# Purpurax/mcaat

Hardware: AMD Instinct MI355X
Metric: k-mers/sec through sdbg_build+cycle_finder, 1B-node graph @ 1/2/4/8 GPUs (higher is better)
Workload: dtype u64

## Files before the change

include/mcaat_gpu.h:

```cpp
#ifndef MCAAT_GPU_H
#define MCAAT_GPU_H
#include <stddef.h>
#include <stdint.h>

#ifdef __cplusplus
extern "C" {
#endif

enum mcaat_status {
    MCAAT_OK = 0,
    MCAAT_E_INVALID = -1,
    MCAAT_E_HIP = -2,
    MCAAT_E_NOMEM = -3,
    MCAAT_E_IO = -4,
    MCAAT_E_CAPACITY = -5
};

typedef struct mcaat_ctx mcaat_ctx;
typedef struct mcaat_reads mcaat_reads;
typedef struct mcaat_graph mcaat_graph;
typedef struct mcaat_cycles mcaat_cycles;
typedef struct mcaat_counts mcaat_counts;
typedef struct mcaat_mapped mcaat_mapped;
typedef struct mcaat_comm mcaat_comm;
// ... 90 lines not shown
                     const uint64_t **offsets, size_t *n_cycles);
int mcaat_cycles_export(const mcaat_cycles *c, uint64_t *sizes, uint64_t *starts, uint64_t *entry_offsets,
                        uint64_t *cycle_offsets, uint64_t *nodes);
int mcaat_cycles_stats(const mcaat_cycles *c, uint64_t *stats);
int mcaat_cycles_candidates(const mcaat_cycles *c, size_t *n, const uint64_t **ids, const int32_t **buckets);
void mcaat_cycles_free(mcaat_cycles *c);

#define MCAAT_COMM_ID_BYTES 128
int mcaat_comm_unique_id(uint8_t *id);
int mcaat_comm_init_rccl(mcaat_ctx *ctx, int world, int rank, const uint8_t *id, mcaat_comm **out);
int mcaat_comm_init_shm(mcaat_ctx *ctx, int world, int rank, const char *name, uint64_t slot_bytes,
                        mcaat_comm **out);
int mcaat_comm_info(const mcaat_comm *c, int *world, int *rank);
int mcaat_comm_schedule_check(int world, uint64_t seed, uint64_t piece_bytes, uint64_t *rounds);
int mcaat_desc_canonical(const uint64_t in[2], int E, uint64_t out[2]);
int mcaat_comm_barrier(mcaat_comm *c);
int mcaat_comm_allgather_sizes(mcaat_comm *c, uint64_t bytes, uint64_t *sizes);
int mcaat_comm_allgatherv(mcaat_comm *c, const void *send, uint64_t bytes, void *recv, const uint64_t *sizes);
void mcaat_comm_free(mcaat_comm *c);
int mcaat_reads_from_fastx_part(mcaat_ctx *ctx, const char *const *files, int n_files, int part, int n_parts,
                                mcaat_reads **out);
int mcaat_reads_file_records(const mcaat_reads *r, int file, uint64_t *n_records);
int mcaat_build_graph_sharded(mcaat_ctx *ctx, mcaat_comm *comm, const mcaat_reads *r, int k, mcaat_graph **out);
int mcaat_cycle_finder_comm(mcaat_graph *g, mcaat_comm *comm, const mcaat_cf_params *p, mcaat_cycles **out);
int mcaat_graph_shard_info(const mcaat_graph *g, int *sharded, uint64_t *first, uint64_t *n_local);
int mcaat_graph_unshard(mcaat_graph *g, mcaat_comm *comm);

int mcaat_stage_times(const mcaat_ctx *ctx, int max, const char **names, double *ms, int *n);
int mcaat_kernel_timing(const mcaat_ctx *ctx, const char *kernel, double *avg_ms, uint64_t *launches,
                        double *bytes_per_launch);
// ... 15 lines not shown
```

mcaat_amd/__init__.py:

```python
from .lib import (
    LIB_PATH,
    CfParams,
    Comm,
    Context,
    Counts,
    CycleResult,
    Graph,
    McaatError,
    Reads,
    SynthSpec,
    count_edges,
    desc_canonical,
    desc_preaggregate,
    edges_reduce,
    device_count,
    load_library,
    preload,
    synth_arrays,
    synth_genome_host,
    synth_host,
)
```

mcaat_amd/csrc/capi.hip:

```cpp
#include <sys/stat.h>
#include <zlib.h>

#include <cstdio>
#include <cstdlib>
#include <cstring>
#include <string>

#include "internal.h"
#include "comm.h"
#include "desc_canon.h"
#include "synth.h"

using namespace mcaat;

namespace {

thread_local std::string g_last_error;

template <class F>
int guarded(F &&f) {
    try {
        f();
        return MCAAT_OK;
    } catch (const Error &e) {
// ... 1026 lines not shown

void mcaat_reset_timing(mcaat_ctx *ctx) {
    if (ctx) ctx->kstats.clear();
}

int mcaat_set_knob(mcaat_ctx *ctx, const char *name, int64_t value) {
    static const char *const known[] = {
        "nc.group_budget", "nc.fallback_budget", "nc.out_cap", "nc.l1_slots", "nc.fine_bits",
        "nc.edge_cap",     "nc.desc_cap",        "sort.msd",   "sort.wave_limit", "sort.mid_limit",
        "sort.block_limit", "cf.dls_stack",      "cf.dls_visited", "cf.fc_lock", "cf.fc_relax",
        "cf.fc_out",       "cf.fc_window",       "cf.walk_budget", "sdbg.adj_lds",   "sdbg.adj_cap",       "cf.ruler_mask",
        "nc.overlap",      "sort.l3_counting",   "cf.peel_list_div", "cf.peel_list_cap", "cf.cand_cap",
        "fq.hostpack",     "sort.mid_counting", "nc.big_table", "cf.fused_init", "sort.mid_occ", "cf.scan_u", "cf.prep_batch", "cf.dls_lanes", "dist.oriented",
        "sort.small_mid", "sort.small_limit", "cf.recount", "cf.dls_host",
        "dist.desc",      "cf.compact",         "cf.fresh",   "cf.dls_persist", "nc.split_first", "nc.split_max", "cf.pull_flags", "cf.dls_budget", "nc.grow_early",
        "nc.free_sync", "dist.shard_cf", "dist.ruler_mask", "dist.adj_chunk", "dist.dir_edges", "nc.ahead", "dist.adj_ranges", "dist.win_ranges", "cf.dls_lds", "cf.dls_lds_cap", "dist.segs_at_one", "nc.a_mini", "dist.bfs_sync", "cf.compact_pct", "dist.bfs_block", "dist.bfs_frontier", "dist.res_fixed", "dist.res_batch", "dist.res_block_mb", "dist.walk_block", "dist.walk_batch", "dist.grid_blocks", "dist.preagg"};
    return guarded([&] {
        require(ctx && name, "null argument");
        bool ok = false;
        for (const char *k : known) ok = ok || strcmp(k, name) == 0;
        if (!ok) throw Error(MCAAT_E_INVALID, std::string("unknown knob: ") + name);
        if (value < 0) ctx->knobs.erase(name);
        else ctx->knobs[name] = value;
    });
}

int mcaat_comm_unique_id(uint8_t *id) {
    return guarded([&] {
        require(id != nullptr, "null argument");
        comm_unique_id(id);
    });
// ... 3 lines not shown
    return guarded([&] {
        const uint64_t r = comm_schedule_check(world, seed, piece_bytes);
        if (rounds) *rounds = r;
    });
}

int mcaat_desc_canonical(const uint64_t in[2], int E, uint64_t out[2]) {
    return guarded([&] {
        require(in && out, "null argument");
        require(E >= 1 && E <= kMaxK + 1, "E must be in [1, 31]");
        require((int)((in[1] >> kNShift) & 63) + E - 1 <= kDescBases, "descriptor longer than its base field");
        uint64_t w0 = in[0], w1 = in[1];
        desc_canonical(w0, w1, E);
        out[0] = w0;
        out[1] = w1;
    });
}

int mcaat_comm_init_rccl(mcaat_ctx *ctx, int world, int rank, const uint8_t *id, mcaat_comm **out) {
    return guarded([&] {
        require(ctx && id && out, "null argument");
        require(world >= 1 && rank >= 0 && rank < world, "rank must be in [0, world)");
        mcaat::bind(ctx);
        auto *c = new mcaat_comm;
        try {
            c->c = comm_rccl(ctx, world, rank, id);
        } catch (...) {
            delete c;
            throw;
        }
// ... 183 lines not shown
```

mcaat_amd/csrc/desc_canon.h:

```cpp
#pragma once
#include <stdint.h>

#if defined(__HIPCC__)
#include <hip/hip_runtime.h>
#define MCAAT_DESC_HD __host__ __device__ __forceinline__
#else
#define MCAAT_DESC_HD inline
#endif

namespace mcaat {

constexpr int kDescBases = 54;
constexpr int kNShift = 44;
constexpr int kHShift = 50;
constexpr int kHBits = 14;

static_assert(kDescBases < 64, "a canonical descriptor's w0 is never all ones only while L < 64");

#if defined(__has_builtin)
#if __has_builtin(__builtin_bitreverse32)
#define MCAAT_DESC_BITREV 1
#endif
#endif
MCAAT_DESC_HD uint32_t desc_rev2_32(uint32_t x) {
#ifdef MCAAT_DESC_BITREV
    const uint32_t y = __builtin_bitreverse32(x);
    return ((y >> 1) & 0x55555555u) | ((y << 1) & 0xAAAAAAAAu);
#else
    x = ((x >> 2) & 0x33333333u) | ((x & 0x33333333u) << 2);
    x = ((x >> 4) & 0x0F0F0F0Fu) | ((x & 0x0F0F0F0Fu) << 4);
    x = ((x >> 8) & 0x00FF00FFu) | ((x & 0x00FF00FFu) << 8);
    return (x >> 16) | (x << 16);
// ... 30 lines not shown
```

mcaat_amd/csrc/node_counter.hip:

```cpp
#include <hipcub/hipcub.hpp>

#include <algorithm>
#include <cstdio>
#include <cstdlib>
#include <ctime>
#include <functional>
#include <memory>
#include <mutex>
#include <type_traits>

#include "desc_canon.h"
#include "internal.h"

namespace mcaat {

namespace {

constexpr int kBlock = 256;


struct SkParams {
    int E;
    int m;
    int w;
    int nmax;
    int l2_bits;
    uint64_t salt;
    uint32_t mini;
};

__device__ __forceinline__ uint64_t desc_window(uint64_t w0, uint64_t w1, int i, int E) {
    uint64_t v;
    if (i == 0) v = w0;
    else if (i < 32) v = (w0 >> (2 * i)) | (w1 << (64 - 2 * i));
    else v = w1 >> (2 * (i - 32));
    return v & mask_bits(2 * E);
}

__device__ __forceinline__ uint32_t rev2_32(uint32_t x) {
    x = ((x >> 2) & 0x33333333u) | ((x & 0x33333333u) << 2);
    x = ((x >> 4) & 0x0F0F0F0Fu) | ((x & 0x0F0F0F0Fu) << 4);
    return __builtin_bswap32(x);
}
// ... 163 lines not shown
#pragma unroll
        for (int t = 0; t < kCk; ++t) hm[t] = min(S[t], Pm[t + W - 1 - kCk]);
    } else {
#pragma unroll
        for (int t = 0; t < kCk; ++t) {
            uint32_t v = at(t);
#pragma unroll
            for (int q = 1; q < W; ++q) v = min(v, at(t + q));
            hm[t] = v;
        }
    }
}

constexpr uint32_t kMiniOne = 1024, kMiniShard = 256;
constexpr uint16_t kDeadSub = 0xffff;


#ifndef MCAAT_WB
#define MCAAT_WB 4
#endif
#ifndef MCAAT_APF
#define MCAAT_APF 1
#endif
[[maybe_unused]] constexpr int kAPF = MCAAT_APF;
constexpr int kWB = MCAAT_WB;
#ifndef MCAAT_WPIPE
#define MCAAT_WPIPE 0
#endif
#ifndef MCAAT_CLOSEMASK
#define MCAAT_CLOSEMASK 1
#endif
constexpr bool kWPipe = MCAAT_WPIPE != 0;

constexpr int kPeP = 7, kPePar = 14, kPeLane = 15;

template <int W, bool FULL>
__global__ void __launch_bounds__(kAThreads) k_sk_scatter(const uint64_t *__restrict__ packed, ItemSrc src,
                                                          SkParams P, uint4 *__restrict__ l1_data,
                                                          const uint64_t *__restrict__ l1_base,
                                                          const uint64_t *__restrict__ l1_cap,
                                                          unsigned long long *l1_cursor, uint16_t *__restrict__ l1_sub,
                                                          unsigned long long *prof, unsigned long long *rstate, int rmode) {
    __shared__ uint64_t stage[kStage];
#if !MCAAT_A1HASH
    __shared__ uint8_t stage_l1[kStage];
#endif
    __shared__ uint16_t perm[kStage];
    __shared__ uint64_t sbase[kAWaves][2][64];
    __shared__ uint32_t hist[256];
    __shared__ uint32_t boff[256];
    __shared__ uint32_t bcur[256];
    __shared__ unsigned long long rpos[256];
    __shared__ unsigned long long rlim[256];
    __shared__ uint32_t rleft[256];
    __shared__ uint32_t wtot[kAWaves];
    __shared__ int more_flag[2];

    const int wave = threadIdx.x >> 6, lane = threadIdx.x & 63;
    const int tb = threadIdx.x;
    unsigned long long my_next = 0, my_base = 0;
    uint32_t prev_need = 0;
    unsigned long long *rs = rstate ? rstate + ((uint64_t)blockIdx.x * 256 + (tb & 255)) * 3 : nullptr;
    if (tb < 256) {
        hist[tb] = 0;
        bcur[tb] = 0;
        my_base = l1_base[tb];
        rlim[tb] = my_base + l1_cap[tb];
        if (rmode >= 2) {
            rpos[tb] = rs[0];
            rleft[tb] = (uint32_t)rs[1];
            my_next = rs[2];
        } else {
            rleft[tb] = 0;
            my_next = atomicAdd(&l1_cursor[tb], (unsigned long long)P.mini);
        }
    }
    if (threadIdx.x == 0) more_flag[0] = more_flag[1] = 0;
    __syncthreads();
    uint64_t *seg = stage + __builtin_amdgcn_readfirstlane(wave * kSeg);
#if !MCAAT_A1HASH
    uint8_t *seg_l1 = stage_l1 + wave * kSeg;
#endif
    uint32_t nflush = 0;

    const int sub_shift = kHShift + kHBits - P.l2_bits;
    auto put = [&](int b, uint64_t pos, const uint4 &d) {
        if (pos < rlim[b]) {
            l1_data[pos] = d;
            const uint64_t hi = (uint64_t)d.w << 32;
            l1_sub[pos] = ((d.w >> (kNShift - 32)) & 63) ? (uint16_t)(sub_shift < 64 ? hi >> sub_shift : 0) : kDeadSub;
        }
    };

    const uint64_t n_items = src.fixed_len ? src.n_reads * src.ipr : src.n_items;
    const uint64_t n_batches = (n_items + 63) / 64;
    const uint64_t bstride = (uint64_t)gridDim.x * kAWaves;
    uint64_t batch = (uint64_t)blockIdx.x * kAWaves + wave;
    constexpr bool kFull = FULL;
    const uint32_t mmask = (uint32_t)mask_bits(2 * P.m);
    const uint32_t salt32 = (uint32_t)P.salt;
    const int nmax = P.nmax;

    uint32_t H[3 * kCk];
#if MCAAT_AREG
    uint32_t iw[kItemRegs - 1];
    u64x2 nraw[3] = {{0, 0}, {0, 0}, {0, 0}};
    uint64_t s1 = 0, s2 = 0;
    int np1 = 0, np2 = 0;
#pragma unroll
    for (int i = 0; i < kItemRegs - 1; ++i) iw[i] = 0;
#else
    uint64_t cw[3], pa = 0, pb = 0;
// ... 247 lines not shown
#endif
        tick(1);
        if (lane == 0) wtot[wave] = fill;
        if (lane == 0 && (active || batch < n_batches)) more_flag[nflush & 1] = 1;
        lds_barrier();
        const int more = more_flag[nflush & 1];
        if (threadIdx.x == 0) more_flag[(nflush + 1) & 1] = 0;
        ++nflush;
        tick(2);
        if (tb < 256) {
            rpos[tb] += prev_need;
            rleft[tb] -= prev_need;
            const uint32_t need = hist[tb];
            if (need > rleft[tb]) {
                for (uint32_t z = 0; z < rleft[tb]; ++z) put(tb, rpos[tb] + z, make_uint4(0, 0, 0, 0));
                if (need <= P.mini) {
                    rpos[tb] = my_base + my_next;
                    rleft[tb] = P.mini;
                    my_next = atomicAdd(&l1_cursor[tb], (unsigned long long)P.mini);
                } else {
                    const uint32_t grab = ((need + P.mini - 1) / P.mini) * P.mini;
                    rpos[tb] = my_base + atomicAdd(&l1_cursor[tb], (unsigned long long)grab);
                    rleft[tb] = grab;
                }
            }
            prev_need = need;
        }
        if (wave == 0) {
            const uint4 hv = *(const uint4 *)&hist[4 * lane];
            const uint32_t sum4 = hv.x + hv.y + hv.z + hv.w;
            uint32_t incl = sum4;
#pragma unroll
            for (int o = 1; o < 64; o <<= 1) {
                const uint32_t v = __shfl_up(incl, o);
                if (lane >= o) incl += v;
            }
// ... 3 lines not shown
        lds_barrier();
        if (tb < 256) hist[tb] = 0;
        tick(3);
        for (uint32_t e = lane; e < fill; e += 64) {
#if MCAAT_A1HASH
            const int b = (int)(*(const uint32_t *)(seg + e) >> 24);
#else
            const int b = seg_l1[e];
#endif
            perm[boff[b] + atomicAdd(&bcur[b], 1u)] = (uint16_t)(wave * kSeg + e);
        }
        lds_barrier();
        uint32_t total = 0;
#pragma unroll
        for (int w = 0; w < kAWaves; ++w) total += wtot[w];
        uint64_t q[2][kWB], B0[2][kWB], x[2][kWB][3];
        auto load_batch = [&](auto Sc, uint32_t j0) {
            constexpr int S = decltype(Sc)::value;
#pragma unroll
            for (int k = 0; k < kWB; ++k) {
                const uint32_t j = j0 + k * kAThreads;
                q[S][k] = 0;
                B0[S][k] = 0;
                if (j < total) {
                    const uint32_t i = perm[j];
                    q[S][k] = stage[i];
                    const uint32_t hi = (uint32_t)(q[S][k] >> 32);
                    const uint32_t ln = (hi >> kPeLane) & 63, pr = (hi >> kPePar) & 1;
                    B0[S][k] = sbase[i / kSeg][pr][ln] + ((hi >> kPeP) & 127);
                }
// ... 54 lines not shown
        if (tb < 256) bcur[tb] = 0;
        fill = 0;
        bsf = active ? 1u : 0u;
        lds_barrier();
        tick(4);
        if (!more) break;
    }
    if (tb < 256) {
        rpos[tb] += prev_need;
        rleft[tb] -= prev_need;
    }
    if (rmode == 1 || rmode == 2) {
        if (tb < 256) {
            rs[0] = rpos[tb];
            rs[1] = rleft[tb];
            rs[2] = my_next;
        }
        return;
    }
    __syncthreads();
    for (int pass = 0; pass < 2; ++pass) {
        for (int b = 0; b < 256; ++b)
            for (uint32_t z = threadIdx.x; z < rleft[b]; z += kAThreads) put(b, rpos[b] + z, make_uint4(0, 0, 0, 0));
        __syncthreads();
        if (tb < 256) {
            rpos[tb] = my_base + my_next;
            rleft[tb] = P.mini;
        }
        __syncthreads();
    }
    if (prof && lane == 0)
        for (int i = 0; i < 5; ++i) atomicAdd(&prof[i], tp[i]);
}

typedef void (*SkKernel)(const uint64_t *, ItemSrc, SkParams, uint4 *, const uint64_t *, const uint64_t *,
                         unsigned long long *, uint16_t *, unsigned long long *, unsigned long long *, int);
SkKernel sk_kernel(int w, bool full) {
    if (full) {
        switch (w) {
#define MCAAT_SK(W) \
    case W:         \
        return k_sk_scatter<W, true>;
            MCAAT_SK(9) MCAAT_SK(10) MCAAT_SK(11) MCAAT_SK(12) MCAAT_SK(13) MCAAT_SK(14) MCAAT_SK(15) MCAAT_SK(16)
#undef MCAAT_SK
        }
    } else {
        switch (w) {
#define MCAAT_SK(W) \
    case W:         \
        return k_sk_scatter<W, false>;
            MCAAT_SK(1) MCAAT_SK(2) MCAAT_SK(3) MCAAT_SK(4) MCAAT_SK(5) MCAAT_SK(6) MCAAT_SK(7) MCAAT_SK(8)
            MCAAT_SK(9) MCAAT_SK(10) MCAAT_SK(11) MCAAT_SK(12) MCAAT_SK(13) MCAAT_SK(14) MCAAT_SK(15) MCAAT_SK(16)
#undef MCAAT_SK
        }
    }
    throw Error(MCAAT_E_INVALID, "node_counter: minimizer window out of range");
}

constexpr int kBThreads = 1024;
constexpr uint32_t kChunk = 65536;


#ifndef MCAAT_BLG
#define MCAAT_BLG 4
#endif
constexpr int kLG = MCAAT_BLG;
static_assert(kLG == 2 || kLG == 4, "32-B or 64-B lines");
__device__ __forceinline__ uint32_t round4(uint32_t x) { return (x + kLG - 1) & ~(uint32_t)(kLG - 1); }

__device__ __forceinline__ void chunk_hist(const uint16_t *__restrict__ sub, uint64_t s0, uint32_t n, uint32_t *lh) {
    const uint4 *v = (const uint4 *)(sub + s0);
    const uint32_t n8 = n / 8;
    for (uint32_t i0 = threadIdx.x; i0 < n8; i0 += 4 * kBThreads) {
        uint4 q[4];
#pragma unroll
// ... 44 lines not shown
    }
}

constexpr int kMaxSub = 2048;
#ifndef MCAAT_BPF
#define MCAAT_BPF 2
#endif
constexpr int kBPF = MCAAT_BPF;
#ifndef MCAAT_BCOOP
#define MCAAT_BCOOP 1
#endif
constexpr bool kCoopFlush = MCAAT_BCOOP != 0;

template <bool WEIGHTED>
__global__ void __launch_bounds__(kBThreads) k_l2_scatter(const uint4 *__restrict__ data,
                                                          const uint16_t *__restrict__ sub,
                                                          const uint64_t *chunk_start, const uint32_t *chunk_len,
                                                          const uint32_t *runs, int l2_bits, int E,
                                                          uint4 *__restrict__ out, uint64_t gbase,
                                                          const uint32_t *__restrict__ wgt,
                                                          uint32_t *__restrict__ out_w) {
    __shared__ uint4 buf[kMaxSub * kLG];
    __shared__ uint32_t lb[kMaxSub];
    __shared__ uint32_t lc[kMaxSub];
    __shared__ uint32_t bl[kMaxSub];
    const uint32_t S = 1u << l2_bits;
    const uint64_t c = blockIdx.x;
    for (uint32_t i = threadIdx.x; i < S; i += kBThreads) {
        lb[i] = runs[c * S + i];
        lc[i] = 0;
        bl[i] = 0;
    }
    __syncthreads();
    const uint64_t s0 = chunk_start[c];
    const uint32_t n = chunk_len[c];
    uint32_t v[kBPF];
    uint4 d[kBPF];
#pragma unroll
    for (int j = 0; j < kBPF; ++j) {
        const uint32_t i = j * kBThreads + threadIdx.x;
        v[j] = i < n ? sub[s0 + i] : kDeadSub;
        d[j] = i < n ? data[s0 + i] : make_uint4(0, 0, 0, 0);
    }
    for (uint32_t i00 = 0; i00 < n; i00 += kBPF * kBThreads)
#pragma unroll
    for (int j = 0; j < kBPF; ++j) {
        const uint32_t i0 = i00 + j * kBThreads;
        if (i0 >= n) break;
        const uint32_t cv = v[j];
        uint4 cd = d[j];
        const uint32_t ni = i0 + kBPF * kBThreads + threadIdx.x;
        v[j] = ni < n ? sub[s0 + ni] : kDeadSub;
        if (ni < n) d[j] = data[s0 + ni];
        const bool live = cv != kDeadSub;
        uint32_t r = 0, line = 0;
        bool buffered = false;
        if (live) {
            r = atomicAdd(&lc[cv], 1u);
            line = bl[cv];
            if constexpr (WEIGHTED) out_w[(uint64_t)lb[cv] * kLG + r - gbase] = wgt[s0 + i0 + threadIdx.x];
            uint64_t w0 = (uint64_t)cd.x | ((uint64_t)cd.y << 32), w1 = (uint64_t)cd.z | ((uint64_t)cd.w << 32);
            desc_canonical(w0, w1, E);
            cd = make_uint4((uint32_t)w0, (uint32_t)(w0 >> 32), (uint32_t)w1, (uint32_t)(w1 >> 32));
            buffered = r / kLG == line;
            if (buffered) buf[cv * kLG + (r & (kLG - 1))] = cd;
            else out[(uint64_t)lb[cv] * kLG + r - gbase] = cd;
        }
        lds_barrier();
        uint32_t nline = 0;
// ... 672 lines not shown
                }
            }
            if (lane == 0) wsum[wave] = wtotal;
            __syncthreads();
            if (threadIdx.x == 0) {
                uint32_t t = 0;
                for (int w = 0; w < kPWaves; ++w) {
                    const uint32_t v = wsum[w];
                    wsum[w] = t;
                    t += v;
                }
                obase = t ? atomicAdd(&rcur[b], (unsigned long long)t) : 0;
                if (raw && t) atomicAdd(&stat[0], (unsigned long long)t);
            }
            __syncthreads();
            const int sub_shift = 64 - l2_bits;
            auto put = [&](uint64_t o, const uint4 &dsc, uint32_t wt) {
                if (o < ocap) {
                    out[ob + o] = dsc;
                    out_w[ob + o] = wt;
                    const uint64_t hi = (uint64_t)dsc.w << 32;
                    out_sub[ob + o] = (uint16_t)(sub_shift < 64 ? hi >> sub_shift : 0);
                    wacc += wt;
                }
            };
            uint64_t o = obase + wsum[wave];
            if (!raw) {
#pragma unroll
                for (int j = 0; j < kPSlots; ++j) {
                    if (c[j]) {
                        const int i = threadIdx.x + j * kPThreads;
                        const unsigned long long w0 = dk0[i], w1 = dk1[i];
                        put(o + __popcll(m[j] & below),
                            make_uint4((uint32_t)w0, (uint32_t)(w0 >> 32), (uint32_t)w1, (uint32_t)(w1 >> 32)), c[j]);
                    }
                    o += __popcll(m[j]);
                }
// ... 92 lines not shown
    const int E = k + 1;
    SkParams P;
    P.E = E;
    P.m = std::max(3, std::min(16, E - 8));
    if (E >= 22) P.m = std::max(14, std::min(16, E - 14));
    if (const char *e = getenv("MCAAT_MINI_W")) {
        const int wt = atoi(e);
        if (wt >= 1 && wt <= 16) P.m = std::max(3, std::min(16, E - wt + 1));
    }
    if (P.m > E) P.m = E;
    P.w = E - P.m + 1;
    if (P.w > 16) throw Error(MCAAT_E_INVALID, "node_counter: minimizer window above 16");
    P.nmax = kDescBases - E + 1;
    P.salt = 0x6d696e696d697aULL;
    P.mini = kMiniOne;

    return P;
}

void node_counter(mcaat_ctx *ctx, const mcaat_reads *r, int k, CountResult &out) {
    NcBuckets b;
    if (r->ahead && r->ahead_k == k) {
        b = std::move(*r->ahead);
        r->ahead.reset();
        verbose_mark(ctx, "node_counter.A_ahead");
    } else {
        node_counter_a(ctx, r, k, nullptr, b);
    }
    node_counter_bc(ctx, b, k, out);
}

// ... 39 lines not shown
            hipLaunchKernelGGL(k_sum_u32, dim3(grid_for(n_items, kBlock, (unsigned)ctx->n_cu * 8)), dim3(kBlock), 0, st,
                               item_np.p, n_items, socc.p);
            LAUNCH_OK();
            unsigned long long h = 0;
            HIP_OK(hipMemcpyAsync(&h, socc.p, 8, hipMemcpyDeviceToHost, st));
            HIP_OK(hipStreamSynchronize(st));
            n_occ = h;
        }
        src.item_base = item_base.p;
        src.item_np = item_np.p;
        src.n_items = n_items;
    }
    const int fine_bits = pick ? pick(n_occ) : nc_fine_bits(ctx, n_occ);
    P.l2_bits = fine_bits - 8;
    if (pick) P.mini = kMiniShard;
    if (knob_set(ctx, "nc.a_mini")) P.mini = (uint32_t)std::max<int64_t>(8, knob(ctx, "nc.a_mini", 1024)) & ~7u;
    bk.l2_bits = P.l2_bits;
    bk.n_occ = n_occ;
    bk.regions.assign(256, {});
    if (n_occ == 0) {
        bk.data.alloc(1);
        bk.sub.alloc(8);
        return;
    }

    const double dens = 2.0 / (P.w + 1);
    uint64_t est = (uint64_t)(1.08 * (dens * (double)n_occ + (double)n_items)) + 4096;
    std::vector<uint64_t> cap(256), base(257);
    const uint64_t a_grid = (uint64_t)kAPerCu * ctx->n_cu;
    for (int b = 0; b < 256; ++b) cap[b] = (est / 256 + 2 * a_grid * P.mini + 7) & ~7ull;
    if (const int64_t fixed = knob(ctx, "nc.l1_slots", 0))
        for (int b = 0; b < 256; ++b) cap[b] = ((uint64_t)fixed + 7) & ~7ull;
    DevBuf<uint64_t> dcap(256), dbase(257);
    DevBuf<unsigned long long> dcur(256);
    DevBuf<uint4> &l1 = bk.data;
    DevBuf<uint16_t> &l1s = bk.sub;
    std::vector<unsigned long long> tot(256);
    static const bool prof_a = getenv("MCAAT_PROF_A") && getenv("MCAAT_PROF_A")[0] == '1';
    DevBuf<unsigned long long> dprof(8);
    if (prof_a) HIP_OK(hipMemsetAsync(dprof.p, 0, dprof.bytes(), st));
    for (int attempt = 0;; ++attempt) {
        base[0] = 0;
        for (int b = 0; b < 256; ++b) base[b + 1] = base[b] + cap[b];
        l1.alloc(base[256]);
        l1s.alloc(base[256]);
        HIP_OK(hipMemcpyAsync(dcap.p, cap.data(), 8 * 256, hipMemcpyHostToDevice, st));
        HIP_OK(hipMemcpyAsync(dbase.p, base.data(), 8 * 257, hipMemcpyHostToDevice, st));
        HIP_OK(hipMemsetAsync(dcur.p, 0, dcur.bytes(), st));
        {
            KernelTimer kt(ctx, "sk_scatter", 0.0);
            hipLaunchKernelGGL(sk_kernel(P.w, P.m == 16), dim3((unsigned)a_grid), dim3(kAThreads), 0, st, r->packed.p, src, P, l1.p,
                               dbase.p, dcap.p, dcur.p, l1s.p, prof_a ? dprof.p : nullptr, nullptr, 0);
            LAUNCH_OK();
            kt.stop();
        }
        HIP_OK(hipMemcpyAsync(tot.data(), dcur.p, 8 * 256, hipMemcpyDeviceToHost, st));
        HIP_OK(hipStreamSynchronize(st));
        bool ok = true;
        for (int b = 0; b < 256; ++b)
            if (tot[b] > cap[b]) ok = false;
        if (ok) break;
        if (attempt > 0) throw Error(MCAAT_E_CAPACITY, "node_counter: L1 bucket sizing failed");
        for (int b = 0; b < 256; ++b) cap[b] = (tot[b] + 8) & ~7ull;
    }
    uint64_t n_desc = 0;
    bk.base = base;
    for (int b = 0; b < 256; ++b) {
        n_desc += tot[b];
        if (tot[b]) bk.regions[b].push_back({base[b], tot[b]});
    }
    ctx->kstats["sk_scatter"].total_bytes += 0.25 * (double)r->n_bases + 18.0 * (double)n_desc;
    if (prof_a) {
        unsigned long long hp[8];
        HIP_OK(hipMemcpy(hp, dprof.p, 64, hipMemcpyDeviceToHost));
        const double waves = (double)a_grid * kAWaves;
        fprintf(stderr, "[mcaat] pass A per-wave ms (100 MHz clock): scan %.1f bucket %.1f wait %.1f reserve %.1f write %.1f\n",
                hp[0] / waves / 1e5, hp[1] / waves / 1e5, hp[2] / waves / 1e5, hp[3] / waves / 1e5, hp[4] / waves / 1e5);
    }
    verbose_mark(ctx, "node_counter.A");
}

struct NcAhead {
    mcaat_ctx *ctx = nullptr;
    int k = 0;
    SkParams P{};
    uint64_t a_grid = 0;
// ... 6 lines not shown
    bool failed = false, ended = false;
    uint64_t n_occ = 0;
    ~NcAhead() {
        if (ctx && !ended) (void)hipStreamSynchronize(ctx->side);
    }
};

static_assert(kItem == kNcItem, "the packer's item estimate uses pass A's item length");

std::shared_ptr<NcAhead> nc_ahead_begin(mcaat_ctx *ctx, int k, uint64_t n_occ_est, uint64_t n_items_est) {
    auto a = std::make_shared<NcAhead>();
    a->ctx = ctx;
    a->k = k;
    a->P = sk_params(k);
    a->P.l2_bits = nc_fine_bits(ctx, n_occ_est) - 8;
    if (knob_set(ctx, "nc.a_mini")) a->P.mini = (uint32_t)std::max<int64_t>(8, knob(ctx, "nc.a_mini", 1024)) & ~7u;
    a->bk = std::make_shared<NcBuckets>();
    a->bk->l2_bits = a->P.l2_bits;
    a->a_grid = (uint64_t)kAPerCu * ctx->n_cu;
    const double dens = 2.0 / (a->P.w + 1);
    const uint64_t est = (uint64_t)(1.12 * (dens * (double)n_occ_est + (double)n_items_est)) + 4096;
    a->cap.assign(256, 0);
    a->base.assign(257, 0);
    for (int b = 0; b < 256; ++b) {
        a->cap[b] = (est / 256 + 2 * a->a_grid * a->P.mini + 7) & ~7ull;
        if (const int64_t fixed = knob(ctx, "nc.l1_slots", 0)) a->cap[b] = ((uint64_t)fixed + 7) & ~7ull;
        a->base[b + 1] = a->base[b] + a->cap[b];
    }
    a->bk->data.alloc(a->base[256]);
    a->bk->sub.alloc(a->base[256]);
    a->dcap.alloc(256);
// ... 7 lines not shown
    return a;
}

void nc_ahead_part(NcAhead &a, const uint64_t *packed, uint64_t n_reads, uint64_t L) {
    const int E = a.k + 1;
    std::lock_guard<std::mutex> g(a.mu);
    if (a.failed || !n_reads || L < (uint64_t)E) return;
    ItemSrc src{};
    src.n_reads = n_reads;
    src.fixed_len = L;
    const uint64_t npos = L - E + 1;
    src.ipr = (npos + kItem - 1) / kItem;
    a.n_occ += n_reads * npos;
    hipLaunchKernelGGL(sk_kernel(a.P.w, a.P.m == 16), dim3((unsigned)a.a_grid), dim3(kAThreads), 0, a.ctx->side, packed,
                       src, a.P, a.bk->data.p, (const uint64_t *)a.dbase.p, (const uint64_t *)a.dcap.p, a.dcur.p,
                       a.bk->sub.p, nullptr, a.state.p, a.launches ? 2 : 1);
    LAUNCH_OK();
    ++a.launches;
}

void nc_ahead_fail(NcAhead &a) {
    std::lock_guard<std::mutex> g(a.mu);
    a.failed = true;
}

std::shared_ptr<NcBuckets> nc_ahead_end(NcAhead &a) {
    std::lock_guard<std::mutex> g(a.mu);
    mcaat_ctx *ctx = a.ctx;
    std::vector<unsigned long long> tot(256, 0);
    if (!a.failed) {
        ItemSrc src{};
        hipLaunchKernelGGL(sk_kernel(a.P.w, a.P.m == 16), dim3((unsigned)a.a_grid), dim3(kAThreads), 0, ctx->side,
                           (const uint64_t *)a.bk->data.p, src, a.P, a.bk->data.p, (const uint64_t *)a.dbase.p,
                           (const uint64_t *)a.dcap.p, a.dcur.p, a.bk->sub.p, nullptr, a.state.p, a.launches ? 3 : 0);
        LAUNCH_OK();
        HIP_OK(hipMemcpyAsync(tot.data(), a.dcur.p, 8 * 256, hipMemcpyDeviceToHost, ctx->side));
    }
    HIP_OK(hipStreamSynchronize(ctx->side));
    a.ended = true;
    for (int b = 0; b < 256 && !a.failed; ++b)
        if (tot[b] > a.cap[b]) a.failed = true;
    if (a.failed) return nullptr;
    NcBuckets &bk = *a.bk;
    bk.n_occ = a.n_occ;
    bk.base = a.base;
    bk.regions.assign(256, {});
    uint64_t n_desc = 0;
    for (int b = 0; b < 256; ++b) {
        n_desc += tot[b];
// ... 129 lines not shown

    const uint32_t dmax = (uint32_t)std::min<int64_t>(kDMax, std::max<int64_t>(1, knob(ctx, "nc.desc_cap", kDMax)));
    const uint32_t split_first = (uint32_t)std::min<int64_t>(kSplitMax, std::max<int64_t>(1, knob(ctx, "nc.split_first", kSplitLg)));
    const uint32_t split_max = (uint32_t)std::min<int64_t>(kSplitMax, std::max<int64_t>(1, knob(ctx, "nc.split_max", kSplitMax)));
    const uint64_t group_budget =
        (uint64_t)knob(ctx, "nc.group_budget", (int64_t)std::max<uint64_t>(hfine[F] / 4 + 1, 1ULL << 28));
    for (int b0 = 0; b0 < 256;) {
        int b1 = b0 + 1;
        while (b1 < 256 && hfine[(uint64_t)(b1 + 1) * S] - hfine[(uint64_t)b0 * S] <= group_budget) ++b1;
        const uint64_t p0 = (uint64_t)b0 * S, p1 = (uint64_t)b1 * S;
        const uint64_t gbase = hfine[p0], gn = hfine[p1] - gbase;
        const uint64_t c0 = plan.bchunk[b0], c1 = plan.bchunk[b1];
        if (gn) {
            DevBuf<uint4> fine(gn);
            {
                KernelTimer kt(ctx, "preagg_partition", 34.0 * (double)gn);
                hipLaunchKernelGGL(k_l2_scatter<false>, dim3((unsigned)(c1 - c0)), dim3(kBThreads), 0, st, bk.data.p, bk.sub.p,
                                   plan.dcs.p + c0, plan.dcl.p + c0, (const uint32_t *)plan.druns.p + c0 * S, bk.l2_bits, E,
                                   fine.p, gbase, (const uint32_t *)nullptr, (uint32_t *)nullptr);
                LAUNCH_OK();
                kt.stop();
            }
            {
                KernelTimer kt(ctx, "desc_preagg", 16.0 * (double)gn);
                const unsigned wg = (unsigned)std::min<uint64_t>(p1 - p0, (uint64_t)kCPerCu * ctx->n_cu);
                hipLaunchKernelGGL(k_desc_preagg, dim3(wg), dim3(kPThreads), 0, st, fine.p, gbase, plan.dfine.p, p0, p1,
                                   bk.l2_bits, out.data.p, out.sub.p, out.wgt.p, (const uint64_t *)drb.p,
                                   (const uint64_t *)drc.p, dcur.p, dmax, split_first, split_max, dstat.p);
                LAUNCH_OK();
                kt.stop();
            }
        }
// ... 94 lines not shown
        hipEvent_t ev = event_get(ctx);
        HIP_OK(hipEventRecord(ev, st));
        HIP_OK(hipStreamWaitEvent(sb, ev, 0));
        event_put(ctx, ev);
    }
    std::vector<KernelTimer *> btimers;
    auto launch_b = [&](Group &g) {
        const uint64_t p0 = (uint64_t)g.b0 * S, p1 = (uint64_t)g.b1 * S;
        const uint64_t gbase = hfine[p0], gn = hfine[p1] - gbase;
        const uint64_t c0 = bchunk[g.b0], c1 = bchunk[g.b1];
        {
            AllocStreamScope scope(sb);
            g.fine.alloc(gn ? gn : 1);
            if (weighted) g.finew.alloc(gn ? gn : 1);
        }
        auto *kt = new KernelTimer(ctx, "l2_partition", 34.0 * (double)gn, sb);
        if (c1 > c0) {
            hipLaunchKernelGGL(weighted ? k_l2_scatter<true> : k_l2_scatter<false>, dim3((unsigned)(c1 - c0)),
                               dim3(kBThreads), 0, sb, l1.p, l1s.p, dcs.p + c0, dcl.p + c0,
                               (const uint32_t *)druns.p + c0 * S, P.l2_bits, E, g.fine.p, gbase,
                               (const uint32_t *)bk.wgt.p, g.finew.p);
            LAUNCH_OK();
        }
        kt->mark();
        g.done = event_get(ctx);
        HIP_OK(hipEventRecord(g.done, sb));
        btimers.push_back(kt);
    };
    struct TimerGuard {
        std::vector<KernelTimer *> &v;
        ~TimerGuard() { for (auto *t : v) delete t; }
    } tguard{btimers};
    uint64_t n_out = 0;
    if (!groups.empty()) launch_b(groups[0]);
// ... 169 lines not shown
```

mcaat_amd/lib.py:

```python
from __future__ import annotations

import ctypes as C
import os
from dataclasses import dataclass, field
from typing import List, Optional, Sequence, Tuple

import numpy as np

LIB_PATH = os.environ.get("MCAAT_LIB") or os.path.join(os.path.dirname(os.path.abspath(__file__)), "libmcaat_gpu.so")

_u64p = C.POINTER(C.c_uint64)
_u32p = C.POINTER(C.c_uint32)
_u16p = C.POINTER(C.c_uint16)
_u8p = C.POINTER(C.c_uint8)
_i32p = C.POINTER(C.c_int32)


class McaatError(RuntimeError):

    def __init__(self, code: int, msg: str):
        super().__init__(f"mcaat error {code}: {msg}")
        self.code = code


# ... 84 lines not shown
    "mcaat_mapped_get": (C.c_int, [C.c_void_p, _u64p, C.POINTER(_u64p), C.POINTER(_u64p), C.POINTER(_u64p)]),
    "mcaat_mapped_free": (None, [C.c_void_p]),
    "mcaat_set_knob": (C.c_int, [C.c_void_p, C.c_char_p, C.c_int64]),
    "mcaat_reads_write_fastq": (C.c_int, [C.c_void_p, C.c_char_p, C.c_int]),
    "mcaat_graph_save": (C.c_int, [C.c_void_p, C.c_char_p]),
    "mcaat_graph_load": (C.c_int, [C.c_void_p, C.c_char_p, C.POINTER(C.c_void_p)]),
    "mcaat_graph_download_range": (C.c_int, [C.c_void_p, C.c_uint64, C.c_uint64, _u64p, _u16p, _u8p]),
    "mcaat_graph_valid_words": (C.c_int, [C.c_void_p, _u64p]),
    "mcaat_graph_keep_region": (C.c_int, [C.c_void_p, _u64p, C.c_size_t, C.c_uint64]),
    "mcaat_graph_succinct_check": (C.c_int, [C.c_void_p, C.c_int, _u64p, C.POINTER(C.c_double)]),
    "mcaat_graph_valid_subgraph": (C.c_int, [C.c_void_p, C.POINTER(C.c_uint64), _u64p, C.POINTER(C.c_uint32),
                                             _u8p]),
    "mcaat_comm_unique_id": (C.c_int, [_u8p]),
    "mcaat_comm_schedule_check": (C.c_int, [C.c_int, C.c_uint64, C.c_uint64, _u64p]),
    "mcaat_desc_canonical": (C.c_int, [_u64p, C.c_int, _u64p]),
    "mcaat_comm_init_rccl": (C.c_int, [C.c_void_p, C.c_int, C.c_int, _u8p, C.POINTER(C.c_void_p)]),
    "mcaat_comm_init_shm": (C.c_int, [C.c_void_p, C.c_int, C.c_int, C.c_char_p, C.c_uint64, C.POINTER(C.c_void_p)]),
    "mcaat_comm_info": (C.c_int, [C.c_void_p, C.POINTER(C.c_int), C.POINTER(C.c_int)]),
    "mcaat_comm_barrier": (C.c_int, [C.c_void_p]),
    "mcaat_comm_allgather_sizes": (C.c_int, [C.c_void_p, C.c_uint64, _u64p]),
    "mcaat_comm_allgatherv": (C.c_int, [C.c_void_p, C.c_void_p, C.c_uint64, C.c_void_p, _u64p]),
    "mcaat_comm_free": (None, [C.c_void_p]),
    "mcaat_reads_from_fastx_part": (C.c_int, [C.c_void_p, C.POINTER(C.c_char_p), C.c_int, C.c_int, C.c_int,
                                              C.POINTER(C.c_void_p)]),
    "mcaat_reads_file_records": (C.c_int, [C.c_void_p, C.c_int, _u64p]),
    "mcaat_build_graph_sharded": (C.c_int, [C.c_void_p, C.c_void_p, C.c_void_p, C.c_int, C.POINTER(C.c_void_p)]),
    "mcaat_cycle_finder_comm": (C.c_int, [C.c_void_p, C.c_void_p, C.POINTER(_CfParams), C.POINTER(C.c_void_p)]),
    "mcaat_desc_preaggregate": (C.c_int, [C.c_void_p, C.c_void_p, C.c_int, _u64p]),
    "mcaat_arena_check": (C.c_int, [C.c_void_p, C.POINTER(C.c_int64)]),
    "mcaat_arena_usage": (C.c_int, [C.c_void_p, C.c_int, _u64p, _u64p, _u64p]),
# ... 28 lines not shown
def _ptr(a: np.ndarray, t):
    return a.ctypes.data_as(t)


def device_count() -> int:
    n = C.c_int(0)
    _check(load_library().mcaat_device_count(C.byref(n)))
    return n.value


def desc_canonical(w0: int, w1: int, E: int) -> Tuple[int, int]:
    src = (C.c_uint64 * 2)(w0, w1)
    dst = (C.c_uint64 * 2)()
    _check(load_library().mcaat_desc_canonical(src, int(E), dst))
    return int(dst[0]), int(dst[1])


def preload(device: int = 0) -> None:
    _check(load_library().mcaat_preload(device))


@dataclass
class SynthSpec:

    seed: int = 1
    n_genomes: int = 1
    genome_len: int = 50_000
    arrays_per_genome: int = 1
    spacers_per_array: int = 12
    repeat_len_min: int = 30
# ... 580 lines not shown
```

Baseline: 146.7 billion.

## Adapt scatter reservation size near tail and derive sub keys from descriptors

```diff
diff --git a/include/mcaat_gpu.h b/include/mcaat_gpu.h
--- a/include/mcaat_gpu.h
+++ b/include/mcaat_gpu.h
@@ -128,6 +128,7 @@
 int mcaat_comm_info(const mcaat_comm *c, int *world, int *rank);
 int mcaat_comm_schedule_check(int world, uint64_t seed, uint64_t piece_bytes, uint64_t *rounds);
 int mcaat_desc_canonical(const uint64_t in[2], int E, uint64_t out[2]);
+int mcaat_desc_sub(uint64_t w1, int l2_bits, int *live, uint32_t *sub);
 int mcaat_comm_barrier(mcaat_comm *c);
 int mcaat_comm_allgather_sizes(mcaat_comm *c, uint64_t bytes, uint64_t *sizes);
 int mcaat_comm_allgatherv(mcaat_comm *c, const void *send, uint64_t bytes, void *recv, const uint64_t *sizes);
diff --git a/mcaat_amd/__init__.py b/mcaat_amd/__init__.py
--- a/mcaat_amd/__init__.py
+++ b/mcaat_amd/__init__.py
@@ -12,6 +12,7 @@
     count_edges,
     desc_canonical,
     desc_preaggregate,
+    desc_sub,
     edges_reduce,
     device_count,
     load_library,
diff --git a/mcaat_amd/csrc/capi.hip b/mcaat_amd/csrc/capi.hip
--- a/mcaat_amd/csrc/capi.hip
+++ b/mcaat_amd/csrc/capi.hip
@@ -1064,7 +1064,7 @@
         "fq.hostpack",     "sort.mid_counting", "nc.big_table", "cf.fused_init", "sort.mid_occ", "cf.scan_u", "cf.prep_batch", "cf.dls_lanes", "dist.oriented",
         "sort.small_mid", "sort.small_limit", "cf.recount", "cf.dls_host",
         "dist.desc",      "cf.compact",         "cf.fresh",   "cf.dls_persist", "nc.split_first", "nc.split_max", "cf.pull_flags", "cf.dls_budget", "nc.grow_early",
-        "nc.free_sync", "dist.shard_cf", "dist.ruler_mask", "dist.adj_chunk", "dist.dir_edges", "nc.ahead", "dist.adj_ranges", "dist.win_ranges", "cf.dls_lds", "cf.dls_lds_cap", "dist.segs_at_one", "nc.a_mini", "dist.bfs_sync", "cf.compact_pct", "dist.bfs_block", "dist.bfs_frontier", "dist.res_fixed", "dist.res_batch", "dist.res_block_mb", "dist.walk_block", "dist.walk_batch", "dist.grid_blocks", "dist.preagg"};
+        "nc.free_sync", "dist.shard_cf", "dist.ruler_mask", "dist.adj_chunk", "dist.dir_edges", "nc.ahead", "dist.adj_ranges", "dist.win_ranges", "cf.dls_lds", "cf.dls_lds_cap", "dist.segs_at_one", "nc.a_mini", "nc.a_adapt", "nc.a_stats", "dist.bfs_sync", "cf.compact_pct", "dist.bfs_block", "dist.bfs_frontier", "dist.res_fixed", "dist.res_batch", "dist.res_block_mb", "dist.walk_block", "dist.walk_batch", "dist.grid_blocks", "dist.preagg"};
     return guarded([&] {
         require(ctx && name, "null argument");
         bool ok = false;
@@ -1098,6 +1098,15 @@
         desc_canonical(w0, w1, E);
         out[0] = w0;
         out[1] = w1;
+    });
+}
+
+int mcaat_desc_sub(uint64_t w1, int l2_bits, int *live, uint32_t *sub) {
+    return guarded([&] {
+        require(live && sub, "null argument");
+        require(l2_bits >= 0 && l2_bits <= kHBits, "l2_bits must be in [0, 14]");
+        *live = desc_live(w1) ? 1 : 0;
+        *sub = desc_sub(w1, l2_bits);
     });
 }
 
diff --git a/mcaat_amd/csrc/desc_canon.h b/mcaat_amd/csrc/desc_canon.h
--- a/mcaat_amd/csrc/desc_canon.h
+++ b/mcaat_amd/csrc/desc_canon.h
@@ -16,6 +16,13 @@
 constexpr int kHBits = 14;
 
 static_assert(kDescBases < 64, "a canonical descriptor's w0 is never all ones only while L < 64");
+
+MCAAT_DESC_HD bool desc_live(uint64_t w1) { return ((w1 >> kNShift) & 63) != 0; }
+
+static_assert(kHShift + kHBits == 64, "the hash bits end at the top of w1");
+MCAAT_DESC_HD uint32_t desc_sub(uint64_t w1, int l2_bits) {
+    return l2_bits > 0 ? (uint32_t)(w1 >> (64 - l2_bits)) : 0u;
+}
 
 #if defined(__has_builtin)
 #if __has_builtin(__builtin_bitreverse32)
diff --git a/mcaat_amd/csrc/node_counter.hip b/mcaat_amd/csrc/node_counter.hip
--- a/mcaat_amd/csrc/node_counter.hip
+++ b/mcaat_amd/csrc/node_counter.hip
@@ -27,6 +27,8 @@
     int l2_bits;
     uint64_t salt;
     uint32_t mini;
+    uint32_t a_epb;
+    uint32_t a_far;
 };
 
 __device__ __forceinline__ uint64_t desc_window(uint64_t w0, uint64_t w1, int i, int E) {
@@ -220,6 +222,13 @@
 
 constexpr uint32_t kMiniOne = 1024, kMiniShard = 256;
 constexpr uint16_t kDeadSub = 0xffff;
+constexpr int kResShift = 44;
+constexpr unsigned long long kResMask = (1ull << kResShift) - 1;
+constexpr uint32_t kMiniMax = 1u << 16;
+#ifndef MCAAT_AADAPTQ
+#define MCAAT_AADAPTQ 8
+#endif
+constexpr uint32_t kAdaptQ = MCAAT_AADAPTQ;
 
 
 #ifndef MCAAT_WB
@@ -246,7 +255,8 @@
                                                           const uint64_t *__restrict__ l1_base,
                                                           const uint64_t *__restrict__ l1_cap,
                                                           unsigned long long *l1_cursor, uint16_t *__restrict__ l1_sub,
-                                                          unsigned long long *prof, unsigned long long *rstate, int rmode) {
+                                                          unsigned long long *prof, unsigned long long *rstate, int rmode,
+                                                          unsigned long long *dstat) {
     __shared__ uint64_t stage[kStage];
 #if !MCAAT_A1HASH
     __shared__ uint8_t stage_l1[kStage];
@@ -265,8 +275,23 @@
     const int wave = threadIdx.x >> 6, lane = threadIdx.x & 63;
     const int tb = threadIdx.x;
     unsigned long long my_next = 0, my_base = 0;
+    uint32_t my_nsz = 0;
     uint32_t prev_need = 0;
     unsigned long long *rs = rstate ? rstate + ((uint64_t)blockIdx.x * 256 + (tb & 255)) * 3 : nullptr;
+    const uint64_t n_items = src.fixed_len ? src.n_reads * src.ipr : src.n_items;
+    const uint64_t n_batches = (n_items + 63) / 64;
+    const uint64_t bstride = (uint64_t)gridDim.x * kAWaves;
+    uint64_t batch = (uint64_t)blockIdx.x * kAWaves + wave;
+    const bool adapt = P.a_epb != 0 && (rmode == 0 || rmode == 3);
+    const uint64_t far_span = (uint64_t)P.a_far * bstride;
+    auto next_size = [&](uint32_t in_hand) -> uint32_t {
+        if (!adapt || batch + far_span <= n_batches) return P.mini;
+        const uint64_t rem = batch < n_batches ? (n_batches - batch + bstride - 1) / bstride : 0;
+        const uint64_t expect = (rem * kAWaves * P.a_epb) >> 8;
+        const uint64_t beyond = expect > in_hand ? expect - in_hand : 0;
+        if (beyond >= P.mini) return P.mini;
+        return min(P.mini, ((uint32_t)(beyond * kAdaptQ / 4) + 64 + 7) & ~7u);
+    };
     if (tb < 256) {
         hist[tb] = 0;
         bcur[tb] = 0;
@@ -275,10 +300,12 @@
         if (rmode >= 2) {
             rpos[tb] = rs[0];
             rleft[tb] = (uint32_t)rs[1];
-            my_next = rs[2];
+            my_next = rs[2] & kResMask;
+            my_nsz = (uint32_t)(rs[2] >> kResShift);
         } else {
             rleft[tb] = 0;
-            my_next = atomicAdd(&l1_cursor[tb], (unsigned long long)P.mini);
+            my_nsz = next_size(0);
+            my_next = atomicAdd(&l1_cursor[tb], (unsigned long long)my_nsz);
         }
     }
     if (threadIdx.x == 0) more_flag[0] = more_flag[1] = 0;
@@ -289,19 +316,14 @@
 #endif
     uint32_t nflush = 0;
 
-    const int sub_shift = kHShift + kHBits - P.l2_bits;
     auto put = [&](int b, uint64_t pos, const uint4 &d) {
         if (pos < rlim[b]) {
             l1_data[pos] = d;
             const uint64_t hi = (uint64_t)d.w << 32;
-            l1_sub[pos] = ((d.w >> (kNShift - 32)) & 63) ? (uint16_t)(sub_shift < 64 ? hi >> sub_shift : 0) : kDeadSub;
+            l1_sub[pos] = desc_live(hi) ? (uint16_t)desc_sub(hi, P.l2_bits) : kDeadSub;
         }
     };
 
-    const uint64_t n_items = src.fixed_len ? src.n_reads * src.ipr : src.n_items;
-    const uint64_t n_batches = (n_items + 63) / 64;
-    const uint64_t bstride = (uint64_t)gridDim.x * kAWaves;
-    uint64_t batch = (uint64_t)blockIdx.x * kAWaves + wave;
     constexpr bool kFull = FULL;
     const uint32_t mmask = (uint32_t)mask_bits(2 * P.m);
     const uint32_t salt32 = (uint32_t)P.salt;
@@ -579,12 +601,14 @@
             const uint32_t need = hist[tb];
             if (need > rleft[tb]) {
                 for (uint32_t z = 0; z < rleft[tb]; ++z) put(tb, rpos[tb] + z, make_uint4(0, 0, 0, 0));
-                if (need <= P.mini) {
+                if (dstat && rleft[tb]) atomicAdd(&dstat[1], (unsigned long long)rleft[tb]);
+                if (need <= my_nsz) {
                     rpos[tb] = my_base + my_next;
-                    rleft[tb] = P.mini;
-                    my_next = atomicAdd(&l1_cursor[tb], (unsigned long long)P.mini);
+                    rleft[tb] = my_nsz;
+                    my_nsz = next_size(my_nsz - need);
+                    my_next = atomicAdd(&l1_cursor[tb], (unsigned long long)my_nsz);
                 } else {
-                    const uint32_t grab = ((need + P.mini - 1) / P.mini) * P.mini;
+                    const uint32_t grab = ((need + my_nsz - 1) / my_nsz) * my_nsz;
                     rpos[tb] = my_base + atomicAdd(&l1_cursor[tb], (unsigned long long)grab);
                     rleft[tb] = grab;
                 }
@@ -618,6 +642,7 @@
         uint32_t total = 0;
 #pragma unroll
         for (int w = 0; w < kAWaves; ++w) total += wtot[w];
+        if (dstat && threadIdx.x == 0 && total) atomicAdd(&dstat[0], (unsigned long long)total);
         uint64_t q[2][kWB], B0[2][kWB], x[2][kWB][3];
         auto load_batch = [&](auto Sc, uint32_t j0) {
             constexpr int S = decltype(Sc)::value;
@@ -702,18 +727,19 @@
         if (tb < 256) {
             rs[0] = rpos[tb];
             rs[1] = rleft[tb];
-            rs[2] = my_next;
+            rs[2] = my_next | ((unsigned long long)my_nsz << kResShift);
         }
         return;
     }
     __syncthreads();
     for (int pass = 0; pass < 2; ++pass) {
+        if (dstat && tb < 256 && rleft[tb]) atomicAdd(&dstat[2], (unsigned long long)rleft[tb]);
         for (int b = 0; b < 256; ++b)
             for (uint32_t z = threadIdx.x; z < rleft[b]; z += kAThreads) put(b, rpos[b] + z, make_uint4(0, 0, 0, 0));
         __syncthreads();
         if (tb < 256) {
             rpos[tb] = my_base + my_next;
-            rleft[tb] = P.mini;
+            rleft[tb] = my_nsz;
         }
         __syncthreads();
     }
@@ -722,7 +748,8 @@
 }
 
 typedef void (*SkKernel)(const uint64_t *, ItemSrc, SkParams, uint4 *, const uint64_t *, const uint64_t *,
-                         unsigned long long *, uint16_t *, unsigned long long *, unsigned long long *, int);
+                         unsigned long long *, uint16_t *, unsigned long long *, unsigned long long *, int,
+                         unsigned long long *);
 SkKernel sk_kernel(int w, bool full) {
     if (full) {
         switch (w) {
@@ -746,7 +773,11 @@
 }
 
 constexpr int kBThreads = 1024;
-constexpr uint32_t kChunk = 65536;
+#ifndef MCAAT_BCHUNK
+#define MCAAT_BCHUNK 65536
+#endif
+constexpr uint32_t kChunk = MCAAT_BCHUNK;
+static_assert(kChunk >= 8 && kChunk % 8 == 0 && kChunk <= (1u << 24), "chunks start on 16-B aligned sub rows");
 
 
 #ifndef MCAAT_BLG
@@ -821,7 +852,6 @@
 
 template <bool WEIGHTED>
 __global__ void __launch_bounds__(kBThreads) k_l2_scatter(const uint4 *__restrict__ data,
-                                                          const uint16_t *__restrict__ sub,
                                                           const uint64_t *chunk_start, const uint32_t *chunk_len,
                                                           const uint32_t *runs, int l2_bits, int E,
                                                           uint4 *__restrict__ out, uint64_t gbase,
@@ -841,12 +871,10 @@
     __syncthreads();
     const uint64_t s0 = chunk_start[c];
     const uint32_t n = chunk_len[c];
-    uint32_t v[kBPF];
     uint4 d[kBPF];
 #pragma unroll
     for (int j = 0; j < kBPF; ++j) {
         const uint32_t i = j * kBThreads + threadIdx.x;
-        v[j] = i < n ? sub[s0 + i] : kDeadSub;
         d[j] = i < n ? data[s0 + i] : make_uint4(0, 0, 0, 0);
     }
     for (uint32_t i00 = 0; i00 < n; i00 += kBPF * kBThreads)
@@ -854,12 +882,12 @@
     for (int j = 0; j < kBPF; ++j) {
         const uint32_t i0 = i00 + j * kBThreads;
         if (i0 >= n) break;
-        const uint32_t cv = v[j];
         uint4 cd = d[j];
         const uint32_t ni = i0 + kBPF * kBThreads + threadIdx.x;
-        v[j] = ni < n ? sub[s0 + ni] : kDeadSub;
-        if (ni < n) d[j] = data[s0 + ni];
-        const bool live = cv != kDeadSub;
+        d[j] = ni < n ? data[s0 + ni] : make_uint4(0, 0, 0, 0);
+        const uint64_t cw1 = (uint64_t)cd.w << 32;
+        const bool live = desc_live(cw1);
+        const uint32_t cv = desc_sub(cw1, l2_bits);
         uint32_t r = 0, line = 0;
         bool buffered = false;
         if (live) {
@@ -1562,13 +1590,11 @@
                 if (raw && t) atomicAdd(&stat[0], (unsigned long long)t);
             }
             __syncthreads();
-            const int sub_shift = 64 - l2_bits;
             auto put = [&](uint64_t o, const uint4 &dsc, uint32_t wt) {
                 if (o < ocap) {
                     out[ob + o] = dsc;
                     out_w[ob + o] = wt;
-                    const uint64_t hi = (uint64_t)dsc.w << 32;
-                    out_sub[ob + o] = (uint16_t)(sub_shift < 64 ? hi >> sub_shift : 0);
+                    out_sub[ob + o] = (uint16_t)desc_sub((uint64_t)dsc.w << 32, l2_bits);
                     wacc += wt;
                 }
             };
@@ -1691,7 +1717,7 @@
     P.nmax = kDescBases - E + 1;
     P.salt = 0x6d696e696d697aULL;
     P.mini = kMiniOne;
-
+    P.a_epb = P.a_far = 0;
     return P;
 }
 
@@ -1761,7 +1787,13 @@
     const int fine_bits = pick ? pick(n_occ) : nc_fine_bits(ctx, n_occ);
     P.l2_bits = fine_bits - 8;
     if (pick) P.mini = kMiniShard;
-    if (knob_set(ctx, "nc.a_mini")) P.mini = (uint32_t)std::max<int64_t>(8, knob(ctx, "nc.a_mini", 1024)) & ~7u;
+    if (knob_set(ctx, "nc.a_mini"))
+        P.mini = (uint32_t)std::min<int64_t>(kMiniMax, std::max<int64_t>(8, knob(ctx, "nc.a_mini", 1024))) & ~7u;
+    if (knob(ctx, "nc.a_adapt", 1) != 0 && n_items) {
+        const double epi = 2.0 / (P.w + 1) * (double)n_occ / (double)n_items + 1.0;
+        P.a_epb = (uint32_t)std::max<int64_t>(1, std::llround(epi * 64.0));
+        P.a_far = (uint32_t)((512ull * P.mini + (uint64_t)kAWaves * P.a_epb - 1) / ((uint64_t)kAWaves * P.a_epb));
+    }
     bk.l2_bits = P.l2_bits;
     bk.n_occ = n_occ;
     bk.regions.assign(256, {});
@@ -1786,6 +1818,8 @@
     static const bool prof_a = getenv("MCAAT_PROF_A") && getenv("MCAAT_PROF_A")[0] == '1';
     DevBuf<unsigned long long> dprof(8);
     if (prof_a) HIP_OK(hipMemsetAsync(dprof.p, 0, dprof.bytes(), st));
+    const bool a_stats = knob(ctx, "nc.a_stats", 0) != 0;
+    DevBuf<unsigned long long> dslots(3);
     for (int attempt = 0;; ++attempt) {
         base[0] = 0;
         for (int b = 0; b < 256; ++b) base[b + 1] = base[b] + cap[b];
@@ -1794,10 +1828,11 @@
         HIP_OK(hipMemcpyAsync(dcap.p, cap.data(), 8 * 256, hipMemcpyHostToDevice, st));
         HIP_OK(hipMemcpyAsync(dbase.p, base.data(), 8 * 257, hipMemcpyHostToDevice, st));
         HIP_OK(hipMemsetAsync(dcur.p, 0, dcur.bytes(), st));
+        if (a_stats) HIP_OK(hipMemsetAsync(dslots.p, 0, dslots.bytes(), st));
         {
             KernelTimer kt(ctx, "sk_scatter", 0.0);
             hipLaunchKernelGGL(sk_kernel(P.w, P.m == 16), dim3((unsigned)a_grid), dim3(kAThreads), 0, st, r->packed.p, src, P, l1.p,
-                               dbase.p, dcap.p, dcur.p, l1s.p, prof_a ? dprof.p : nullptr, nullptr, 0);
+                               dbase.p, dcap.p, dcur.p, l1s.p, prof_a ? dprof.p : nullptr, nullptr, 0, a_stats ? dslots.p : nullptr);
             LAUNCH_OK();
             kt.stop();
         }
@@ -1817,6 +1852,14 @@
         if (tot[b]) bk.regions[b].push_back({base[b], tot[b]});
     }
     ctx->kstats["sk_scatter"].total_bytes += 0.25 * (double)r->n_bases + 18.0 * (double)n_desc;
+    if (a_stats) {
+        unsigned long long hs[3];
+        d2h(ctx, hs, dslots.p, 24);
+        ctx->kstats["a_slots_reserved"].launches += n_desc;
+        ctx->kstats["a_slots_live"].launches += hs[0];
+        ctx->kstats["a_slots_dead_switch"].launches += hs[1];
+        ctx->kstats["a_slots_dead_end"].launches += hs[2];
+    }
     if (prof_a) {
         unsigned long long hp[8];
         HIP_OK(hipMemcpy(hp, dprof.p, 64, hipMemcpyDeviceToHost));
@@ -1853,7 +1896,8 @@
     a->k = k;
     a->P = sk_params(k);
     a->P.l2_bits = nc_fine_bits(ctx, n_occ_est) - 8;
-    if (knob_set(ctx, "nc.a_mini")) a->P.mini = (uint32_t)std::max<int64_t>(8, knob(ctx, "nc.a_mini", 1024)) & ~7u;
+    if (knob_set(ctx, "nc.a_mini"))
+        a->P.mini = (uint32_t)std::min<int64_t>(kMiniMax, std::max<int64_t>(8, knob(ctx, "nc.a_mini", 1024))) & ~7u;
     a->bk = std::make_shared<NcBuckets>();
     a->bk->l2_bits = a->P.l2_bits;
     a->a_grid = (uint64_t)kAPerCu * ctx->n_cu;
@@ -1891,7 +1935,7 @@
     a.n_occ += n_reads * npos;
     hipLaunchKernelGGL(sk_kernel(a.P.w, a.P.m == 16), dim3((unsigned)a.a_grid), dim3(kAThreads), 0, a.ctx->side, packed,
                        src, a.P, a.bk->data.p, (const uint64_t *)a.dbase.p, (const uint64_t *)a.dcap.p, a.dcur.p,
-                       a.bk->sub.p, nullptr, a.state.p, a.launches ? 2 : 1);
+                       a.bk->sub.p, nullptr, a.state.p, a.launches ? 2 : 1, nullptr);
     LAUNCH_OK();
     ++a.launches;
 }
@@ -1909,7 +1953,7 @@
         ItemSrc src{};
         hipLaunchKernelGGL(sk_kernel(a.P.w, a.P.m == 16), dim3((unsigned)a.a_grid), dim3(kAThreads), 0, ctx->side,
                            (const uint64_t *)a.bk->data.p, src, a.P, a.bk->data.p, (const uint64_t *)a.dbase.p,
-                           (const uint64_t *)a.dcap.p, a.dcur.p, a.bk->sub.p, nullptr, a.state.p, a.launches ? 3 : 0);
+                           (const uint64_t *)a.dcap.p, a.dcur.p, a.bk->sub.p, nullptr, a.state.p, a.launches ? 3 : 0, nullptr);
         LAUNCH_OK();
         HIP_OK(hipMemcpyAsync(tot.data(), a.dcur.p, 8 * 256, hipMemcpyDeviceToHost, ctx->side));
     }
@@ -2069,8 +2113,8 @@
         if (gn) {
             DevBuf<uint4> fine(gn);
             {
-                KernelTimer kt(ctx, "preagg_partition", 34.0 * (double)gn);
-                hipLaunchKernelGGL(k_l2_scatter<false>, dim3((unsigned)(c1 - c0)), dim3(kBThreads), 0, st, bk.data.p, bk.sub.p,
+                KernelTimer kt(ctx, "preagg_partition", 32.0 * (double)gn);
+                hipLaunchKernelGGL(k_l2_scatter<false>, dim3((unsigned)(c1 - c0)), dim3(kBThreads), 0, st, bk.data.p,
                                    plan.dcs.p + c0, plan.dcl.p + c0, (const uint32_t *)plan.druns.p + c0 * S, bk.l2_bits, E,
                                    fine.p, gbase, (const uint32_t *)nullptr, (uint32_t *)nullptr);
                 LAUNCH_OK();
@@ -2195,10 +2239,10 @@
             g.fine.alloc(gn ? gn : 1);
             if (weighted) g.finew.alloc(gn ? gn : 1);
         }
-        auto *kt = new KernelTimer(ctx, "l2_partition", 34.0 * (double)gn, sb);
+        auto *kt = new KernelTimer(ctx, "l2_partition", 32.0 * (double)gn, sb);
         if (c1 > c0) {
             hipLaunchKernelGGL(weighted ? k_l2_scatter<true> : k_l2_scatter<false>, dim3((unsigned)(c1 - c0)),
-                               dim3(kBThreads), 0, sb, l1.p, l1s.p, dcs.p + c0, dcl.p + c0,
+                               dim3(kBThreads), 0, sb, l1.p, dcs.p + c0, dcl.p + c0,
                                (const uint32_t *)druns.p + c0 * S, P.l2_bits, E, g.fine.p, gbase,
                                (const uint32_t *)bk.wgt.p, g.finew.p);
             LAUNCH_OK();
diff --git a/mcaat_amd/lib.py b/mcaat_amd/lib.py
--- a/mcaat_amd/lib.py
+++ b/mcaat_amd/lib.py
@@ -122,6 +122,7 @@
     "mcaat_comm_unique_id": (C.c_int, [_u8p]),
     "mcaat_comm_schedule_check": (C.c_int, [C.c_int, C.c_uint64, C.c_uint64, _u64p]),
     "mcaat_desc_canonical": (C.c_int, [_u64p, C.c_int, _u64p]),
+    "mcaat_desc_sub": (C.c_int, [C.c_uint64, C.c_int, C.POINTER(C.c_int), C.POINTER(C.c_uint32)]),
     "mcaat_comm_init_rccl": (C.c_int, [C.c_void_p, C.c_int, C.c_int, _u8p, C.POINTER(C.c_void_p)]),
     "mcaat_comm_init_shm": (C.c_int, [C.c_void_p, C.c_int, C.c_int, C.c_char_p, C.c_uint64, C.POINTER(C.c_void_p)]),
     "mcaat_comm_info": (C.c_int, [C.c_void_p, C.POINTER(C.c_int), C.POINTER(C.c_int)]),
@@ -180,6 +181,13 @@
     dst = (C.c_uint64 * 2)()
     _check(load_library().mcaat_desc_canonical(src, int(E), dst))
     return int(dst[0]), int(dst[1])
+
+
+def desc_sub(w1: int, l2_bits: int) -> Tuple[bool, int]:
+    live = C.c_int(0)
+    sub = C.c_uint32(0)
+    _check(load_library().mcaat_desc_sub(int(w1), int(l2_bits), C.byref(live), C.byref(sub)))
+    return bool(live.value), int(sub.value)
 
 
 def preload(device: int = 0) -> None:
```

After: 148.6 billion, median of 6. +1.3%, better.
